# FerrisMind/candle-video

Measured on AMD Instinct MI355X. Metric: frames/sec end-to-end LTX-Video-2B 512x768x97; DiT step ms; VAE decode ms, higher is better.
Workload: dtype bf16; 1 GPU; LTX-Video-0.9.8-2B-distilled 512x768x97, 7 steps (configs.rs:223-240), untiled VAE decode; preset=0.9.8-2b-distilled, denoise_steps=7, parallelism=replicas x1 (no data-path collective)

## Files before the change

candle-video_amd/csrc/gemm_asm.hip:

```cpp
#include <atomic>
#include <cstdlib>
#include <cstring>
#include "gemm_common.h"
#include "options.h"

namespace {

typedef float f32x32 __attribute__((ext_vector_type(32)));
typedef uint32_t u32x16 __attribute__((ext_vector_type(16)));
typedef uint32_t u32x8 __attribute__((ext_vector_type(8)));
typedef uint32_t u32x2 __attribute__((ext_vector_type(2)));
#ifndef GEMM_ASM_LOOP_INC
#define GEMM_ASM_LOOP_INC "gemm_asm_loop.inc"
#endif
#include GEMM_ASM_LOOP_INC

extern __shared__ __attribute__((aligned(16))) unsigned char asm_smem[];

#ifdef LTX_EXPERIMENTS
template <int BM, int BN, int WGM, int WGN> struct AsmLoop;
template <> struct AsmLoop<256, 256, 2, 2> {
    template <typename... T> static __device__ __forceinline__ void run(f32x32 (&c)[10], T&&... t) { gemm_asm_loop_256_256(c[0], c[1], c[2], c[3], c[4], c[5], c[6], c[7], t...); }
};
template <> struct AsmLoop<320, 256, 2, 2> {
    template <typename... T> static __device__ __forceinline__ void run(f32x32 (&c)[10], T&&... t) { gemm_asm_loop_320_256(c[0], c[1], c[2], c[3], c[4], c[5], c[6], c[7], c[8], c[9], t...); }
};
template <> struct AsmLoop<160, 256, 1, 4> {
    template <typename... T> static __device__ __forceinline__ void run(f32x32 (&c)[10], T&&... t) { gemm_asm_loop_160_256(c[0], c[1], c[2], c[3], c[4], t...); }
};

template <int BM, int BN, int WGM, int WGN, int EPI>
__global__ __launch_bounds__(256, 1) void gemm_asm_kernel(const GemmArgs g) {
    constexpr int WM = BM / WGM, WN = BN / WGN, MB = WM / 32, NB = WN / 32, NT = MB * NB, AI = BM / 32, BI = BN / 32;
    constexpr int STAGE = (BM + BN) * 128;
    const int tid = threadIdx.x, lane = tid & 63, wave = __builtin_amdgcn_readfirstlane(tid >> 6);
    const int r = lane & 31, h = lane >> 5;
    const int wm = wave / WGN, wn = wave % WGN;
    const int ntn = (g.N + BN - 1) / BN;
    int bid = blockIdx.x;
    if (g.xcd_remap) {
        const int nblk = (int)gridDim.x, q = nblk >> 3, rr = nblk & 7, x = bid & 7, i = bid >> 3;
        bid = (x < rr ? x * (q + 1) : rr * (q + 1) + (x - rr) * q) + i;
    }
    int mt, nt;
    if (g.group_m > 1) {
        const int ntm = (g.M + BM - 1) / BM, gsz = g.group_m * ntn;
        const int grp = bid / gsz, w = bid - grp * gsz, gm0 = grp * g.group_m;
        const int rows = ntm - gm0 < g.group_m ? ntm - gm0 : g.group_m;
        nt = w / rows; mt = gm0 + (w - nt * rows);
    } else { mt = bid / ntn; nt = bid - mt * ntn; }
    const int m0 = mt * BM, n0 = nt * BN;

#ifndef GEMM_ASM_REG
#define GEMM_ASM_REG 0
#endif
    constexpr bool REGSTAGE = GEMM_ASM_REG && BM == 256 && BN == 256;
// ... 37 lines not shown
    const uint32_t ldsw = (uint32_t)__builtin_amdgcn_readfirstlane((int)(smem_base + (uint32_t)wave * 1024u));
    const int nk = __builtin_amdgcn_readfirstlane(g.K / 64);

    f32x32 c[10];
    AsmLoop<BM, BN, WGM, WGN>::run(c, rbase, dma0, dma1, ra, rw, nk, 0u, 0u, ldsw);

#pragma unroll
    for (int t = 0; t < NT; ++t) {
        const int nb = t / MB, mb = t - nb * MB;
        const int m = m0 + wm * WM + mb * 32 + r;
        if (m >= g.M) continue;
#pragma unroll
        for (int g4 = 0; g4 < 4; ++g4) {
            const int n = n0 + wn * WN + nb * 32 + 8 * g4 + 4 * h;
            if (n >= g.N) continue;
            const int e = (t & 1) * 16 + 4 * g4;
            float v[4] = {c[t >> 1][e], c[t >> 1][e + 1], c[t >> 1][e + 2], c[t >> 1][e + 3]};
            epilogue<bf16_t, EPI>(g, m, n, v);
        }
    }
}

#endif

template <int BM, int BN, int WGM, int WGN> struct AsmLoop16;
template <> struct AsmLoop16<256, 256, 2, 2> {
    template <typename... T> static __device__ __forceinline__ void run(f32x32 (&c)[10], const u32x8& rb, const u32x16& d0, const u32x2&, T&&... t) {
        gemm_asm16_loop_256_256(c[0], c[1], c[2], c[3], c[4], c[5], c[6], c[7], rb, d0, t...); }
    static __device__ __forceinline__ void store(int p, int wm, const f32x32 (&c)[10], const u32x8& ad) {
        if (wm == p) gemm_asm16_store_256_256_p0(c[0], c[1], c[2], c[3], c[4], c[5], c[6], c[7], ad); }
};
template <> struct AsmLoop16<160, 256, 1, 4> {
    template <typename... T> static __device__ __forceinline__ void run(f32x32 (&c)[10], const u32x8& rb, const u32x16& d0, const u32x2&, T&&... t) {
        gemm_asm16_loop_160_256(c[0], c[1], c[2], c[3], c[4], rb, d0, t...); }
    static __device__ __forceinline__ void store(int p, int, const f32x32 (&c)[10], const u32x8& ad) {
        if (p == 0) gemm_asm16_store_160_256_p0(c[0], c[1], c[2], c[3], c[4], ad); else gemm_asm16_store_160_256_p1(c[0], c[1], c[2], c[3], c[4], ad); }
    template <typename... T> static __device__ __forceinline__ void run_res(f32x32 (&c)[10], u32x16 (&res)[5], const u32x2& rvoff, const u32x4& rres, uint32_t rstride,
                                                                            const u32x8& rb, const u32x16& d0, T&&... t) {
        gemm_asm16_loop_160_256_res(c[0], c[1], c[2], c[3], c[4], rb, d0, t..., res[0], res[1], res[2], res[3], res[4], rvoff, rres, rstride); }
};
template <> struct AsmLoop16<320, 256, 2, 2> {
    template <typename... T> static __device__ __forceinline__ void run(f32x32 (&c)[10], const u32x8& rb, const u32x16& d0, const u32x2& d1, T&&... t) {
        gemm_asm16_loop_320_256(c[0], c[1], c[2], c[3], c[4], c[5], c[6], c[7], c[8], c[9], rb, d0, d1, t...); }
    static __device__ __forceinline__ void store(int p, int wm, const f32x32 (&c)[10], const u32x8& ad) {
        if (wm != (p >> 1)) return;
        if ((p & 1) == 0) gemm_asm16_store_320_256_p0(c[0], c[1], c[2], c[3], c[4], c[5], c[6], c[7], c[8], c[9], ad);
        else gemm_asm16_store_320_256_p1(c[0], c[1], c[2], c[3], c[4], c[5], c[6], c[7], c[8], c[9], ad); }
};

#ifdef GEMM_ASM_TRACE
__device__ uint32_t g_asm16_trace[1024 * 4 * 16];
#endif

template <int BM, int BN, int WGM, int WGN, int EPI, bool RSQ = false, bool PF_R = false, bool FOLD = false>
__global__ __launch_bounds__(256, 1) void gemm_asm16_kernel(const GemmArgs g) {
    constexpr int WM = BM / WGM, WN = BN / WGN, MB = WM / 16, NB = WN / 16, NT = MB * NB, AI = BM / 32, BI = BN / 32;
    constexpr int STAGE = (BM + BN) * 128;
#ifdef GEMM_ASM_TRACE
    const uint32_t t_entry = (uint32_t)wall_clock64();
#endif
#ifndef ASM16_NO_KERNARG_BATCH
    asm volatile("" :: "s"(g.A), "s"(g.W), "s"(g.M), "s"(g.N), "s"(g.K), "s"(g.lda), "s"(g.xcd_remap), "s"(g.group_m), "s"(g.rows_per_batch), "s"(gridDim.x));
#endif
    const int tid = threadIdx.x, lane = tid & 63, wave = __builtin_amdgcn_readfirstlane(tid >> 6);
    const int rr = lane & 15, q = lane >> 4;
    const int wm = wave / WGN, wn = wave % WGN;
    const int ntn = (g.N + BN - 1) / BN;
    int bid = blockIdx.x;
    if (g.xcd_remap) {
        const int nblk = (int)gridDim.x, qq = nblk >> 3, r8 = nblk & 7, x = bid & 7, i = bid >> 3;
        bid = (x < r8 ? x * (qq + 1) : r8 * (qq + 1) + (x - r8) * qq) + i;
    }
    int mt, nt;
    if (g.group_m > 1) {
        const int ntm = (g.M + BM - 1) / BM, gsz = g.group_m * ntn;
        const int grp = bid / gsz, w = bid - grp * gsz, gm0 = grp * g.group_m;
        const int rows = ntm - gm0 < g.group_m ? ntm - gm0 : g.group_m;
        nt = w / rows; mt = gm0 + (w - nt * rows);
    } else { mt = bid / ntn; nt = bid - mt * ntn; }
    const int m0 = mt * BM, n0 = nt * BN;
    static_assert(!FOLD || BM <= 256 || BM == 320, "norm fold: 64 extra rows = 256 (row, group) units");
    f32x4 fpt[4], fpx = {0.f, 0.f, 0.f, 0.f};
    if constexpr (FOLD) {
        auto group_of = [&](int row, int q4) {
            const int m = m0 + row < g.M ? m0 + row : g.M - 1;
            const bool in = 4 * q4 < g.rs_n;
            const f32x4 u = *reinterpret_cast<const f32x4*>(g.rs_sq + (int64_t)m * g.rs_n + (in ? 4 * q4 : g.rs_n - 4));
            return in ? u : (f32x4){0.f, 0.f, 0.f, 0.f};
        };
        const int row = tid < BM ? tid : BM - 1;
#pragma unroll
        for (int q4 = 0; q4 < 4; ++q4) fpt[q4] = group_of(row, q4);
        if constexpr (BM > 256) fpx = group_of(256 + (tid >> 2), tid & 3);
    }
    const int lr = lane >> 3, pc = lane & 7;
    u32x16 dma0; u32x2 dma1 = {0x80000000u, 0x80000000u};
#pragma unroll
    for (int j = 0; j < 16; ++j) dma0[j] = 0x80000000u;
    auto set_piece = [&](int j, uint32_t v) { if (j < 16) dma0[j] = v; else dma1[j - 16] = v; };
#pragma unroll
    for (int j = 0; j < AI; ++j) {
        const int row = 8 * (j * 4 + wave) + lr;
        int m = m0 + row; if (m > g.M - 1) m = g.M - 1;
#ifdef ASM16_NOSWZ
        set_piece(j, ((uint32_t)m * (uint32_t)g.lda + (uint32_t)pc * 8u) * 2u);
#else
        set_piece(j, ((uint32_t)m * (uint32_t)g.lda + (uint32_t)(pc ^ ((row >> 1) & 7)) * 8u) * 2u);
#endif
    }
#pragma unroll
    for (int j = 0; j < BI; ++j) {
        const int row = 8 * (j * 4 + wave) + lr;
        int n = n0 + row; if (n > g.N - 1) n = g.N - 1;
#ifdef ASM16_NOSWZ
        set_piece(AI + j, ((uint32_t)n * (uint32_t)g.K + (uint32_t)pc * 8u) * 2u);
#else
        set_piece(AI + j, ((uint32_t)n * (uint32_t)g.K + (uint32_t)(pc ^ ((row >> 1) & 7)) * 8u) * 2u);
#endif
    }
    const uint32_t smem_base = (uint32_t)(uintptr_t)(__attribute__((address_space(3))) unsigned char*)asm_smem;
    u32x8 rbase;
#pragma unroll
    for (int st = 0; st < 2; ++st)
#pragma unroll
        for (int kh = 0; kh < 2; ++kh) {
            const uint32_t ch = (uint32_t)(((4 * kh + q) ^ ((rr >> 1) & 7)) << 4);
            rbase[st * 2 + kh] = smem_base + st * STAGE + BM * 128 + (wn * WN + rr) * 128 + ch;
            rbase[4 + st * 2 + kh] = smem_base + st * STAGE + (wm * WM + rr) * 128 + ch;
        }
    const uint64_t ap = (uint64_t)(uintptr_t)g.A, wp = (uint64_t)(uintptr_t)g.W;
    const u32x4 ra = {(uint32_t)__builtin_amdgcn_readfirstlane((int)(uint32_t)ap), (uint32_t)__builtin_amdgcn_readfirstlane((int)(uint32_t)(ap >> 32)) & 0xffffu, 0x80000000u, 0x00020000u};
    const u32x4 rw = {(uint32_t)__builtin_amdgcn_readfirstlane((int)(uint32_t)wp), (uint32_t)__builtin_amdgcn_readfirstlane((int)(uint32_t)(wp >> 32)) & 0xffffu, 0x80000000u, 0x00020000u};
    const uint32_t ldsw = (uint32_t)__builtin_amdgcn_readfirstlane((int)(smem_base + (uint32_t)wave * 1024u));
    const int nk = __builtin_amdgcn_readfirstlane(g.K / 64);
    f32x32 c[10];
    constexpr bool HAS_R = EPI == EPI_GATE_RESID || EPI == EPI_RESID;
    constexpr int RP = BM == 256 ? 128 : 80;
    static_assert(!PF_R || (HAS_R && BM == 160 && BN == 256), "residual prefetch: the 160 x 256 tile's residual epilogues");
    u32x16 pf[5];
    u32x2 pf_voff = {0x80000000u, 0x80000000u}; u32x4 pf_rsrc = {0u, 0u, 0u, 0u}; uint32_t pf_stride = 0u;
    if constexpr (PF_R) {
        const int rows_valid_pf = g.M - m0 < BM ? g.M - m0 : BM;
        const uint64_t rp = (uint64_t)(uintptr_t)(reinterpret_cast<const bf16_t*>(g.resid) + (int64_t)m0 * g.ldr + n0);
        pf_rsrc = (u32x4){(uint32_t)__builtin_amdgcn_readfirstlane((int)(uint32_t)rp), (uint32_t)__builtin_amdgcn_readfirstlane((int)(uint32_t)(rp >> 32)) & 0xffffu,
                          (uint32_t)__builtin_amdgcn_readfirstlane((int)(((uint32_t)(rows_valid_pf - 1) * (uint32_t)g.ldr + 256u) * 2u)), 0x00020000u};
        const int cg_pf = tid & 31;
        const uint32_t row0 = (uint32_t)(tid >> 5) * (uint32_t)g.ldr * 2u;
        pf_voff[0] = n0 + 4 * cg_pf < g.N ? row0 + (uint32_t)(8 * cg_pf) : 0x80000000u;
        pf_voff[1] = n0 + 4 * cg_pf + 128 < g.N ? row0 + (uint32_t)(8 * cg_pf + 256) : 0x80000000u;
        pf_stride = (uint32_t)__builtin_amdgcn_readfirstlane((int)(8u * (uint32_t)g.ldr * 2u));
    }
    if constexpr (FOLD) {
        __builtin_amdgcn_sched_barrier(0);
        asm volatile("" : "+v"(fpt[0]), "+v"(fpt[1]), "+v"(fpt[2]), "+v"(fpt[3]), "+v"(fpx), "+v"(dma0), "+v"(dma1), "+v"(rbase));
        float* rl = reinterpret_cast<float*>(asm_smem + 2 * STAGE);
        if (tid < BM) {
            float ss = 0.f;
#pragma unroll
            for (int q4 = 0; q4 < 4; ++q4) { ss += fpt[q4][0]; ss += fpt[q4][1]; ss += fpt[q4][2]; ss += fpt[q4][3]; }
            rl[tid] = 1.0f / sqrtf(ss * (1.0f / (float)g.rs_D) + g.rs_eps);
        }
        if constexpr (BM > 256) {
            float run = 0.f;
#pragma unroll
            for (int q4 = 0; q4 < 4; ++q4) {
                const float before = q4 ? __shfl(run, (lane & ~3) + q4 - 1) : 0.f;
                if ((tid & 3) == q4) { run = before; run += fpx[0]; run += fpx[1]; run += fpx[2]; run += fpx[3]; }
            }
            if ((tid & 3) == 3) rl[256 + (tid >> 2)] = 1.0f / sqrtf(run * (1.0f / (float)g.rs_D) + g.rs_eps);
        }
    }
#ifdef ASM16_STAGGER
    const uint32_t k0 = (uint32_t)__builtin_amdgcn_readfirstlane((int)(((unsigned)blockIdx.x % ASM16_STAGGER) * (unsigned)(nk / ASM16_STAGGER) * 128u));
#else
    const uint32_t k0 = 0u;
#endif
#ifdef GEMM_ASM_TRACE
    uint32_t tr[8];
    const uint32_t t_loop0 = (uint32_t)wall_clock64();
    AsmLoop16<BM, BN, WGM, WGN>::run(c, rbase, dma0, dma1, ra, rw, nk, k0, k0, ldsw, (uint32_t)__builtin_amdgcn_readfirstlane(g.K * 2), tr);
    const uint32_t t_loop1 = (uint32_t)wall_clock64();
#else
    if constexpr (PF_R) AsmLoop16<BM, BN, WGM, WGN>::run_res(c, pf, pf_voff, pf_rsrc, pf_stride, rbase, dma0, ra, rw, nk, k0, k0, ldsw, (uint32_t)__builtin_amdgcn_readfirstlane(g.K * 2));
    else AsmLoop16<BM, BN, WGM, WGN>::run(c, rbase, dma0, dma1, ra, rw, nk, k0, k0, ldsw, (uint32_t)__builtin_amdgcn_readfirstlane(g.K * 2));
#endif
// ... 174 lines not shown
                            float* lf = reinterpret_cast<float*>(asm_smem + RP * 1024) + (2 * row) * 36 + cg;
                            lf[0] = lA; lf[36] = lB;
                        } else {
                            float* rowf = reinterpret_cast<float*>(asm_smem + row * 1024);
                            rowf[(cg ^ (row & 15)) << 2] = lA;
                            rowf[((cg + 32) ^ (row & 15)) << 2] = lB;
                        }
                    }
                }
            }
            if constexpr (RSQ) {
                __syncthreads();
                const int ng = (g.N + 127) >> 7;
#pragma unroll 1
                for (int pi = tid; pi < RP * 2; pi += 256) {
                    const int row = pi >> 1, half = pi & 1, sw = row & 15;
                    float sum;
                    if constexpr (RSQ_COMPACT) {
                        const f32x4* lf = reinterpret_cast<const f32x4*>(reinterpret_cast<const float*>(asm_smem + RP * 1024) + pi * 36);
                        f32x4 t[8];
#pragma unroll
                        for (int c4 = 0; c4 < 8; ++c4) t[c4] = lf[c4];
                        sum = t[0][0]; sum += t[0][1]; sum += t[0][2]; sum += t[0][3];
#pragma unroll
                        for (int c4 = 1; c4 < 8; ++c4) { sum += t[c4][0]; sum += t[c4][1]; sum += t[c4][2]; sum += t[c4][3]; }
                    } else {
                        const float* rowf = reinterpret_cast<const float*>(asm_smem + row * 1024);
                        sum = rowf[((32 * half) ^ sw) << 2];
#pragma unroll
                        for (int c2 = 1; c2 < 32; ++c2) sum += rowf[((c2 + 32 * half) ^ sw) << 2];
                    }
                    const int trow = p * RP + row, ncol = n0 + 128 * half;
                    if (m0 + trow < g.M && ncol < g.N) g.rowsq[(int64_t)(m0 + trow) * ng + (ncol >> 7)] = sum;
                }
            }
        }
        };
        if (straddle) run_passes(std::true_type{}); else run_passes(std::false_type{});
#ifdef GEMM_ASM_TRACE
        if (lane == 0 && blockIdx.x < 1024) { uint32_t* o = g_asm16_trace + (blockIdx.x * 4 + wave) * 16; o[13] = t_e0; o[14] = t_e1; o[15] = t_e2; }
#endif
    }
#ifdef GEMM_ASM_TRACE
    asm volatile("s_waitcnt vmcnt(0)" ::: "memory");
    if (lane == 0 && blockIdx.x < 1024) {
        uint32_t* o = g_asm16_trace + (blockIdx.x * 4 + wave) * 16;
        for (int i = 0; i < 8; ++i) o[i] = tr[i];
        uint32_t hwid; asm volatile("s_getreg_b32 %0, hwreg(HW_REG_HW_ID)" : "=s"(hwid));
        o[8] = t_entry; o[9] = t_loop0; o[10] = t_loop1; o[11] = (uint32_t)wall_clock64(); o[12] = hwid;
    }
#endif
}

template <int EPI>
__global__ __launch_bounds__(256, 1) void gemm_asm16_conv_kernel(const GemmArgs g) {
    constexpr int BM = 256, BN = 256, WGN = 2, WM = 128, WN = 128, NB = 8, AI = 8, BI = 8, STAGE = (BM + BN) * 128, RP = 128;
    const int tid = threadIdx.x, lane = tid & 63, wave = __builtin_amdgcn_readfirstlane(tid >> 6);
    const int rr = lane & 15, q = lane >> 4;
    const int wm = wave / WGN, wn = wave % WGN;
    const int ntn = (g.N + BN - 1) / BN;
    const int sf = g.sk_sf > 1 ? g.sk_sf : 1;
    const int tile = (int)blockIdx.x / sf, part = (int)blockIdx.x - tile * sf;
    const int mt = tile / ntn, nt = tile - mt * ntn;
    const int m0 = mt * BM, n0 = nt * BN;
    const int KC = g.Cin / 64, nk = g.ntaps * KC;
    const int kt0 = (int)((int64_t)part * nk / sf), kt1 = (int)((int64_t)(part + 1) * nk / sf);
    const int per_it = 9 * KC, it0 = kt0 / per_it, r2 = kt0 - it0 * per_it, kc0 = r2 / 9, hw0 = r2 - kc0 * 9, ih0 = hw0 / 3, iw0 = hw0 - ih0 * 3;
    const int64_t m_base = m0 > 2 * g.H * g.Wd + g.Wd + 1 ? (int64_t)m0 - (2 * g.H * g.Wd + g.Wd + 1) : 0;
    const int lr = lane >> 3, pc = lane & 7;
    const uint32_t frame_bytes = (uint32_t)g.H * (uint32_t)g.Wd * (uint32_t)g.Cin * 2u;
    u32x16 dma0; u32x8 ab[3], vmask;
#pragma unroll
    for (int j = 0; j < AI; ++j) {
        const int row = 8 * (j * 4 + wave) + lr;
        int m = m0 + row; if (m > g.M - 1) m = g.M - 1;
        const int w = m % g.Wd, t1 = m / g.Wd, h = t1 % g.H, t = (t1 / g.H) % g.T;
        vmask[j] = (uint32_t)((h > 0 ? 1 : 0) | 2 | (h < g.H - 1 ? 4 : 0) | (w > 0 ? 8 : 0) | 16 | (w < g.Wd - 1 ? 32 : 0));
        const uint32_t a_off = ((uint32_t)(m - m_base) * (uint32_t)g.Cin + (uint32_t)(pc ^ ((row >> 1) & 7)) * 8u) * 2u;
#pragma unroll
        for (int i = 0; i < 3; ++i) {
            int tt = t + (it0 + i) - g.pad_t; tt = tt < 0 ? 0 : (tt > g.T - 1 ? g.T - 1 : tt);
            ab[i][j] = a_off + (uint32_t)(tt - t) * frame_bytes;
        }
        dma0[j] = 0x80000000u;
    }
#pragma unroll
    for (int j = 0; j < BI; ++j) {
        const int row = 8 * (j * 4 + wave) + lr;
        int n = n0 + row; if (n > g.N - 1) n = g.N - 1;
        dma0[AI + j] = ((uint32_t)n * (uint32_t)g.K + (uint32_t)(pc ^ ((row >> 1) & 7)) * 8u) * 2u;
    }
    const uint32_t smem_base = (uint32_t)(uintptr_t)(__attribute__((address_space(3))) unsigned char*)asm_smem;
    u32x8 rbase;
#pragma unroll
    for (int st = 0; st < 2; ++st)
#pragma unroll
        for (int kh = 0; kh < 2; ++kh) {
            const uint32_t ch = (uint32_t)(((4 * kh + q) ^ ((rr >> 1) & 7)) << 4);
            rbase[st * 2 + kh] = smem_base + st * STAGE + BM * 128 + (wn * WN + rr) * 128 + ch;
            rbase[4 + st * 2 + kh] = smem_base + st * STAGE + (wm * WM + rr) * 128 + ch;
        }
    const uint64_t ap = (uint64_t)(uintptr_t)(reinterpret_cast<const bf16_t*>(g.A) + m_base * g.Cin), wp = (uint64_t)(uintptr_t)g.W;
    const u32x4 ra = {(uint32_t)__builtin_amdgcn_readfirstlane((int)(uint32_t)ap), (uint32_t)__builtin_amdgcn_readfirstlane((int)(uint32_t)(ap >> 32)) & 0xffffu, 0x80000000u, 0x00020000u};
    const u32x4 rw = {(uint32_t)__builtin_amdgcn_readfirstlane((int)(uint32_t)wp), (uint32_t)__builtin_amdgcn_readfirstlane((int)(uint32_t)(wp >> 32)) & 0xffffu, 0x80000000u, 0x00020000u};
    const uint32_t ldsw = (uint32_t)__builtin_amdgcn_readfirstlane((int)(smem_base + (uint32_t)wave * 1024u));
    const uint32_t cinb = (uint32_t)g.Cin * 2u, rowb = (uint32_t)g.Wd * cinb, nk2 = (uint32_t)g.N * (uint32_t)g.K * 2u;
// ... 94 lines not shown
        __syncthreads();
        if (*flag == 0u) return;
        const float* base = g.sk_ws + (int64_t)tile * sf * (BM * BN);
        constexpr int UR = 4;
#pragma unroll 1
        for (int k0 = 0; k0 < BM / 8; k0 += UR) {
            f32x4 vA[UR], vB[UR];
            bf16x4 qA[UR] = {}, qB[UR] = {};
#pragma unroll
            for (int j = 0; j < UR; ++j) {
                const int trow = r0 + 8 * (k0 + j);
                int m = m0 + trow; if (m > g.M - 1) m = g.M - 1;
                const float* rp = base + trow * BN + 4 * cg;
                vA[j] = *reinterpret_cast<const f32x4*>(rp); vB[j] = *reinterpret_cast<const f32x4*>(rp + 128);
                if constexpr (EPI == EPI_RESID) {
                    const bf16_t* rrow = reinterpret_cast<const bf16_t*>(g.resid) + (int64_t)m * g.ldr;
                    if (nA < g.N) qA[j] = *reinterpret_cast<const bf16x4*>(rrow + nA);
                    if (nB < g.N) qB[j] = *reinterpret_cast<const bf16x4*>(rrow + nB);
                }
            }
            for (int pq = 1; pq < sf; ++pq) {
#pragma unroll
                for (int j = 0; j < UR; ++j) {
                    const float* rp = base + (int64_t)pq * (BM * BN) + (r0 + 8 * (k0 + j)) * BN + 4 * cg;
                    vA[j] += *reinterpret_cast<const f32x4*>(rp); vB[j] += *reinterpret_cast<const f32x4*>(rp + 128);
                }
            }
#pragma unroll
            for (int j = 0; j < UR; ++j) {
                const int m = m0 + r0 + 8 * (k0 + j);
                if (m >= g.M) continue;
                float a4[4] = {vA[j][0], vA[j][1], vA[j][2], vA[j][3]}, b4[4] = {vB[j][0], vB[j][1], vB[j][2], vB[j][3]};
                if constexpr (EPI == EPI_D2S) {
                    if (nA < g.N) epilogue<bf16_t, EPI>(g, m, nA, a4);
                    if (nB < g.N) epilogue<bf16_t, EPI>(g, m, nB, b4);
                } else {
                    bf16_t* crow = reinterpret_cast<bf16_t*>(g.C) + (int64_t)m * g.ldc;
                    if (nA < g.N) {
                        for (int i = 0; i < 4; ++i) a4[i] += bA4[i];
                        if constexpr (EPI == EPI_RESID) for (int i = 0; i < 4; ++i) a4[i] += (float)qA[j][i];
                        store4<bf16_t>(crow + nA, a4);
                    }
                    if (nB < g.N) {
                        for (int i = 0; i < 4; ++i) b4[i] += bB4[i];
                        if constexpr (EPI == EPI_RESID) for (int i = 0; i < 4; ++i) b4[i] += (float)qB[j][i];
                        store4<bf16_t>(crow + nB, b4);
                    }
                }
            }
        }
    }
}

struct AsmTile { int bm, bn; const char* name; };
const AsmTile kAsmTiles[] = {{256, 256, "asm256x256"}, {320, 256, "asm320x256"}, {160, 256, "asm160x256"}};

template <int BM, int BN, int WGM, int WGN, int EPI, bool MF16 = false>
int launch_asm(const GemmArgs& g, hipStream_t s) {
    constexpr int smem = 2 * (BM + BN) * 128;
    static std::atomic<unsigned long long> attr_devs{0}, attr_devs_rsq{0};
    void (*kern)(const GemmArgs);
#ifdef LTX_EXPERIMENTS
    if constexpr (MF16) kern = gemm_asm16_kernel<BM, BN, WGM, WGN, EPI>; else kern = gemm_asm_kernel<BM, BN, WGM, WGN, EPI>;
#else
    static_assert(MF16, "the 32x32x16 kernel is an experiment build's");
    kern = gemm_asm16_kernel<BM, BN, WGM, WGN, EPI>;
#endif
    bool wrote_rowsq = false;
    constexpr bool CAN_PF = MF16 && BM == 160 && BN == 256 && (EPI == EPI_GATE_RESID || EPI == EPI_RESID);
    bool pf_r = false;
    if constexpr (CAN_PF) pf_r = g.K / 64 >= 12 && ltx_exp("gemm_asm16_resid_prefetch", 1);
    if constexpr (MF16 && (EPI == EPI_BIAS || EPI == EPI_GATE_RESID || EPI == EPI_RESID)) {
        if (g.rowsq) { kern = gemm_asm16_kernel<BM, BN, WGM, WGN, EPI, true>; wrote_rowsq = true; }
    }
    static std::atomic<unsigned long long> attr_devs_pf{0}, attr_devs_pf_rsq{0};
    if constexpr (CAN_PF) {
        if (pf_r) kern = g.rowsq ? gemm_asm16_kernel<BM, BN, WGM, WGN, EPI, true, true> : gemm_asm16_kernel<BM, BN, WGM, WGN, EPI, false, true>;
    }
    static std::atomic<unsigned long long> attr_devs_fold{0};
    bool fold_in = false;
    if constexpr (MF16 && (EPI == EPI_BIAS || EPI == EPI_GELU)) {
        if (g.rs_sq) {
            if (g.rowsq || !g.cvec || g.rs_n < 4 || g.rs_n > 16 || g.rs_n % 4 || g.rows_per_batch < 1) LTX_FAIL(LTX_ERR_ARG, "gemm_asm16: norm fold needs cvec, 4 .. 16 row partials in groups of four and no rowsq by-product");
            kern = gemm_asm16_kernel<BM, BN, WGM, WGN, EPI, false, false, true>; fold_in = true;
        }
    } else if (g.rs_sq) LTX_FAIL(LTX_ERR_ARG, "gemm_asm16: norm fold (rs_sq) on an epilogue that does not carry it");
    if (g.C2 && !(wrote_rowsq && (EPI == EPI_GATE_RESID || EPI == EPI_RESID))) LTX_FAIL(LTX_ERR_ARG, "gemm_asm16: the second output (C2) rides on the residual epilogues with rowsq");
    const int smem_l = smem + (fold_in ? 2048 : 0);
    LTX_TRY(ltx_set_max_dyn_smem(fold_in ? attr_devs_fold : pf_r ? (wrote_rowsq ? attr_devs_pf_rsq : attr_devs_pf) : (wrote_rowsq ? attr_devs_rsq : attr_devs), reinterpret_cast<const void*>(kern), smem_l));
    GemmArgs ga = g;
    ga.xcd_remap = ltx_exp("xcd_remap", 1);
    {
        const int C = 32;
        int gm = 1; while ((gm + 1) * (gm + 1) * BM <= C * BN) ++gm;
        { const int x_gm = ltx_exp("gemm_group_m", -1); if (x_gm >= 0) gm = x_gm; }
        const int ntm = cdiv(g.M, BM);
        if (gm > ntm) gm = ntm;
        ga.group_m = gm < 2 ? 0 : gm;
    }
    const int tiles = cdiv(g.M, BM) * cdiv(g.N, BN);
    LTX_LAUNCH_TIMED(kern, dim3((unsigned)tiles), dim3(256), smem_l, s, ga);
    LTX_CHECK_LAUNCH();
    if (wrote_rowsq) ltx_gemm_rowsq_done();
    return LTX_OK;
}

template <int BM, int BN, int WGM, int WGN, bool MF16 = false>
int launch_asm_epi(const GemmArgs& g, int epi, hipStream_t s) {
    switch (epi) {
        case EPI_BIAS: return launch_asm<BM, BN, WGM, WGN, EPI_BIAS, MF16>(g, s);
        case EPI_GELU: return launch_asm<BM, BN, WGM, WGN, EPI_GELU, MF16>(g, s);
        case EPI_GATE_RESID: return launch_asm<BM, BN, WGM, WGN, EPI_GATE_RESID, MF16>(g, s);
        case EPI_RESID: return launch_asm<BM, BN, WGM, WGN, EPI_RESID, MF16>(g, s);
    }
    LTX_FAIL(LTX_ERR_ARG, "gemm_asm: bad epilogue");
}

}

bool ltx_gemm_asm16_fits(const GemmArgs& g, int epi) {
    if (g.conv || g.pn_on) return false;
    if (epi != EPI_BIAS && epi != EPI_GELU && epi != EPI_GATE_RESID && epi != EPI_RESID) return false;
    if (g.K < 128 || g.K % 64 != 0 || g.lda % 8 != 0 || ((uintptr_t)g.A & 15) || ((uintptr_t)g.W & 15)) return false;
    if ((double)g.M * g.lda * 2.0 >= 2147483648.0 || (double)g.N * g.K * 2.0 >= 2147483648.0) return false;
    const bool seg_ok = !g.c_seg_shift || ((1 << g.c_seg_shift) % 256 == 0 && g.c_seg_stride % 4 == 0);
    if ((double)g.ldc * 2.0 * 320.0 >= 2147483648.0 || (double)g.ldr * 2.0 * 320.0 >= 2147483648.0) return false;
    if (g.N % 8 != 0 || g.ldc % 4 != 0 || ((uintptr_t)g.C & 7) || !seg_ok) return false;
    if (g.bias && ((uintptr_t)g.bias & 7)) return false;
    if ((epi == EPI_GATE_RESID || epi == EPI_RESID) && (!g.resid || g.ldr % 4 != 0 || ((uintptr_t)g.resid & 7))) return false;
    if (epi == EPI_GATE_RESID && (!g.gate || ((uintptr_t)g.gate & 15) || g.gate_stride % 4 != 0 || g.rows_per_batch < 320)) return false;
    if (ltx_gemm_split_factor(g) > 1) return false;
    return g.M > 512 && g.N >= 512;
}

bool ltx_gemm_fold_ok(const GemmArgs& g, int epi) {
    if (!ltx_gemm_asm16_fits(g, epi) || (ltx_opt().gemm_off & LTX_FAM_ASM16) || !ltx_opt().gemm_wide_epi) return false;
    if (ltx_gemm_route_kind(g, LTX_DT_BF16, epi) != LTX_ROUTE_PLAN) return false;
    if (g.C2) {
        if ((epi != EPI_GATE_RESID && epi != EPI_RESID) || !g.rowsq || !g.scale2 || g.scale2_stride % 4 || ((uintptr_t)g.scale2 & 15) || ((uintptr_t)g.C2 & 7) || g.rows_per_batch < 320 || g.c_seg_shift) return false;
    }
    if (g.rs_sq) {
        if ((epi != EPI_BIAS && epi != EPI_GELU) || g.rowsq || !g.cvec || g.cvec_stride % 4 || ((uintptr_t)g.cvec & 15) || g.rs_n < 4 || g.rs_n > 16 || g.rs_n % 4 || ((uintptr_t)g.rs_sq & 15) || g.rows_per_batch < 320) return false;
    }
    return true;
}

bool ltx_gemm_asm_eligible(const GemmArgs& g, int dtype, int epi) {
#ifdef LTX_EXPERIMENTS
    if (dtype != LTX_DT_BF16 || g.conv || ltx_exp("gemm_asm", 0) != 1) return false;
    if (epi != EPI_BIAS && epi != EPI_GELU && epi != EPI_GATE_RESID && epi != EPI_RESID) return false;
    if (g.K < 128 || g.K % 64 != 0 || g.lda % 8 != 0 || ((uintptr_t)g.A & 15) || ((uintptr_t)g.W & 15)) return false;
    if ((double)g.M * g.lda * 2.0 >= 2147483648.0 || (double)g.N * g.K * 2.0 >= 2147483648.0) return false;
    if (ltx_gemm_split_factor(g) > 1) return false;
    return g.M >= 2048 && g.N >= 1024;
#else
    (void)g; (void)dtype; (void)epi;
    return false;
#endif
}

int ltx_gemm_asm_pick_tile(int M, int N) {
    { const int f = ltx_exp("gemm_asm_tile", -1); if (f >= 0 && f < 3) return f; }
    double best = 1e30; int bi = 0;
    for (int i = 0; i < 3; ++i) {
        const int64_t tiles = (int64_t)cdiv(M, kAsmTiles[i].bm) * cdiv(N, kAsmTiles[i].bn);
        const double cost = (double)cdiv64(tiles, 256) * (double)(kAsmTiles[i].bm * kAsmTiles[i].bn);
        if (cost < best * 0.999) { best = cost; bi = i; }
    }
    return bi;
}
const char* ltx_gemm_asm_tile_name(int i) { return i >= 0 && i < 3 ? kAsmTiles[i].name : ""; }

#ifdef GEMM_ASM_TRACE
extern "C" int ltx_dbg_gemm_asm16_trace(uint32_t* out, int n_words) {
    return hipMemcpyFromSymbol(out, HIP_SYMBOL(g_asm16_trace), (size_t)n_words * 4) == hipSuccess ? 0 : -1;
}
#endif

int ltx_launch_gemm_asm16(const GemmArgs& g, int epi, int tile, hipStream_t s) {
    if (((epi == EPI_GATE_RESID && g.gate) || g.C2 || g.rs_sq) && g.rows_per_batch < 320)
        LTX_FAIL(LTX_ERR_ARG, "gemm_asm16: per-group epilogue vectors need groups of at least 320 rows (a tile may meet one group boundary)");
    ltx_prof_kernel(LTX_PROFK_GEMM_ASM16);
    switch (tile) {
        case 0: return launch_asm_epi<256, 256, 2, 2, true>(g, epi, s);
        case 1: return launch_asm_epi<320, 256, 2, 2, true>(g, epi, s);
        case 2: return launch_asm_epi<160, 256, 1, 4, true>(g, epi, s);
    }
    LTX_FAIL(LTX_ERR_ARG, "gemm_asm16: unsupported tile");
}

bool ltx_gemm_asm16_conv_fits(const GemmArgs& g, int epi) {
    if (!g.conv || g.ntaps != 27 || g.kh != 3 || g.kw != 3 || g.pn_on || g.c_seg_shift || g.rowsq) return false;
    if (epi != EPI_BIAS && epi != EPI_RESID && epi != EPI_D2S) return false;
    if (g.Cin % 64 != 0 || g.K != g.Cin || g.N % 8 != 0 || ((uintptr_t)g.A & 15) || ((uintptr_t)g.W & 15) || ((uintptr_t)g.C & 7)) return false;
    if (g.bias && ((uintptr_t)g.bias & 7)) return false;
    if (epi == EPI_RESID && (!g.resid || g.ldr % 4 != 0 || ((uintptr_t)g.resid & 7) || g.ldc % 4 != 0)) return false;
    if (epi == EPI_BIAS && g.ldc % 4 != 0) return false;
    if (epi == EPI_D2S && (g.Cf % 4 != 0 || g.N != 8 * g.Cf)) return false;
    if ((double)g.N * g.K * 2.0 * 10.0 >= 4294967296.0) return false;
    return g.M > 512 && g.N >= 1024 && ltx_gemm_big_fits(g);
}

int ltx_launch_gemm_asm16_conv(const GemmArgs& g, int epi, hipStream_t s) {
    if (!ltx_gemm_asm16_conv_fits(g, epi)) LTX_FAIL(LTX_ERR_ARG, "gemm_asm16 (conv): shape not eligible");
    ltx_prof_kernel(LTX_PROFK_GEMM_ASM16);
    constexpr int smem = 2 * (256 + 256) * 128;
    static std::atomic<unsigned long long> devs[3] = {{0}, {0}, {0}};
    void (*kern)(const GemmArgs) = epi == EPI_BIAS ? gemm_asm16_conv_kernel<EPI_BIAS> : (epi == EPI_RESID ? gemm_asm16_conv_kernel<EPI_RESID> : gemm_asm16_conv_kernel<EPI_D2S>);
    LTX_TRY(ltx_set_max_dyn_smem(devs[epi == EPI_BIAS ? 0 : (epi == EPI_RESID ? 1 : 2)], reinterpret_cast<const void*>(kern), smem));
    GemmArgs ga = g;
    const int tiles = cdiv(g.M, 256) * cdiv(g.N, 256);
    LTX_TRY(ltx_gemm_split_workspace(&ga, tiles, 256, 256, s));
    const int sf = ga.sk_sf > 1 ? ga.sk_sf : 1;
    LTX_LAUNCH_TIMED(kern, dim3((unsigned)(tiles * sf)), dim3(256), smem, s, ga);
    LTX_CHECK_LAUNCH();
    return LTX_OK;
}

int ltx_launch_gemm_asm(const GemmArgs& g, int epi, hipStream_t s) {
#ifdef LTX_EXPERIMENTS
    ltx_prof_kernel(LTX_PROFK_GEMM_ASM);
    switch (ltx_gemm_asm_pick_tile(g.M, g.N)) {
        case 0: return launch_asm_epi<256, 256, 2, 2>(g, epi, s);
        case 1: return launch_asm_epi<320, 256, 2, 2>(g, epi, s);
// ... 8 lines not shown
```

candle-video_amd/csrc/options.cpp:

```cpp
#include "options.h"
#include <atomic>
#include <cstdio>
#include <cstdlib>
#include <cstring>
#include <map>
#include <mutex>
#include <string>
#include "errors.h"

namespace {
std::mutex g_mu;
LtxOptions g_opt;
std::atomic<bool> g_loaded{false};
std::map<std::string, int> g_exp;

struct ListBit { const char* name; unsigned bit; };
const ListBit kFam[] = {{"asm16", LTX_FAM_ASM16}, {"ring", LTX_FAM_RING}, {"p8", LTX_FAM_P8}, {"halo", LTX_FAM_HALO}, {"halo_out", LTX_FAM_HALO_OUT}, {"big", LTX_FAM_BIG}};
const ListBit kAttn[] = {{"q64", LTX_ATTN_Q64}, {"q128", LTX_ATTN_Q128}, {"cross", LTX_ATTN_CROSS}, {"pipe", LTX_ATTN_PIPE}};

template <size_t N> bool parse_list(const char* v, const ListBit (&tab)[N], unsigned* out) {
    unsigned bits = 0;
    std::string s(v ? v : "");
    size_t p = 0;
    while (p < s.size()) {
        size_t q = s.find('+', p); if (q == std::string::npos) q = s.size();
        const std::string item = s.substr(p, q - p);
        bool ok = item.empty();
        for (const auto& t : tab) if (item == t.name) { bits |= t.bit; ok = true; }
        if (!ok) return false;
        p = q + 1;
    }
    *out = bits;
    return true;
}

struct IntField { const char* name; int LtxOptions::*field; };
const IntField kInts[] = {
    {"gemm_tune", &LtxOptions::gemm_tune}, {"gemm_wide_epi", &LtxOptions::gemm_wide_epi}, {"gemm_trace", &LtxOptions::gemm_trace},
    {"attn_q64_big", &LtxOptions::attn_q64_big}, {"vae_tile_batch", &LtxOptions::vae_tile_batch}, {"prof_kernel_events", &LtxOptions::prof_kernel_events}, {"ff2_defer", &LtxOptions::ff2_defer},
    {"gemm_splitk", &LtxOptions::gemm_splitk}, {"q2_fold", &LtxOptions::q2_fold}, {"norm_presum", &LtxOptions::norm_presum}, {"norm_lean", &LtxOptions::norm_lean},
    {"xattn_compact", &LtxOptions::xattn_compact}, {"dense_qkv", &LtxOptions::dense_qkv}, {"vae_fuse_norm", &LtxOptions::vae_fuse_norm}, {"t5_attn_mfma", &LtxOptions::t5_attn_mfma}, {"guidance_batch", &LtxOptions::guidance_batch}, {"norm_fold", &LtxOptions::norm_fold}, {"norm_fold_copies", &LtxOptions::norm_fold_copies}, {"attn_q64_stream", &LtxOptions::attn_q64_stream},
};

bool set_one(LtxOptions& o, const std::string& key, const char* value) {
    static const LtxOptions dflt;
    for (const auto& f : kInts) if (key == f.name) {
        if (!value) { o.*(f.field) = dflt.*(f.field); return true; }
        char* end = nullptr; const long v = strtol(value, &end, 10);
        if (end == value || *end) return false;
        o.*(f.field) = (int)v; return true;
    }
    if (key == "gemm_plan") {
        if (!value) { o.gemm_plan[0] = 0; return true; }
        if (strlen(value) >= sizeof(o.gemm_plan)) return false;
        strcpy(o.gemm_plan, value); return true;
    }
    if (key == "gemm_off") return value ? parse_list(value, kFam, &o.gemm_off) : (o.gemm_off = 0, true);
    if (key == "attn_off") return value ? parse_list(value, kAttn, &o.attn_off) : (o.attn_off = 0, true);
    if (key.rfind("x_", 0) == 0) {
        if (!value) { g_exp.erase(key); return true; }
        char* end = nullptr; const long v = strtol(value, &end, 10);
        if (end == value || *end) return false;
        g_exp[key] = (int)v; return true;
    }
    return false;
}

bool parse_string(LtxOptions& o, const char* text, std::string* bad) {
    std::string s(text ? text : "");
    size_t p = 0;
    while (p < s.size()) {
        size_t q = s.find(',', p); if (q == std::string::npos) q = s.size();
        const std::string item = s.substr(p, q - p);
        p = q + 1;
        if (item.empty()) continue;
        const size_t eq = item.find('=');
        if (eq == std::string::npos || !set_one(o, item.substr(0, eq), item.c_str() + eq + 1)) { if (bad) *bad = item; return false; }
    }
    return true;
}

void load_locked() {
    g_opt = LtxOptions(); g_exp.clear();
    std::string bad;
    if (!parse_string(g_opt, getenv("LTX_OPTIONS"), &bad))
        fprintf(stderr, "[ltx] LTX_OPTIONS: entry '%s' not understood (see include/ltxhip.h); it and what follows it are ignored\n", bad.c_str());
    g_loaded.store(true, std::memory_order_release);
}
}

const LtxOptions& ltx_opt() {
// ... 51 lines not shown
```

candle-video_amd/csrc/options.h:

```cpp
#pragma once

enum { LTX_FAM_ASM16 = 1, LTX_FAM_RING = 2, LTX_FAM_P8 = 4, LTX_FAM_HALO = 8, LTX_FAM_HALO_OUT = 16, LTX_FAM_BIG = 32 };
enum { LTX_ATTN_Q64 = 1, LTX_ATTN_Q128 = 2, LTX_ATTN_CROSS = 4, LTX_ATTN_PIPE = 8 };

struct LtxOptions {
    int gemm_tune = 1;
    char gemm_plan[40] = {0};
    unsigned gemm_off = 0;
    int gemm_wide_epi = 1;
    int gemm_trace = 0;
    int attn_q64_big = -1;
    int vae_tile_batch = 0;
    int prof_kernel_events = 1;
    int ff2_defer = 1;
    int gemm_splitk = 1;
    int q2_fold = 1;
    int norm_presum = 1;
    int norm_lean = 1;
    int xattn_compact = 1;
    int attn_q64_stream = 0;
    int norm_fold = 2;
    int norm_fold_copies = 10;
    int guidance_batch = 1;
    int dense_qkv = 1;
    int vae_fuse_norm = 1;
    int t5_attn_mfma = 1;
    unsigned attn_off = 0;
};

const LtxOptions& ltx_opt();
int ltx_exp_lookup(const char* name, int dflt);
#ifdef LTX_EXPERIMENTS
#define ltx_exp(name, dflt) ltx_exp_lookup(name, dflt)
#else
#define ltx_exp(name, dflt) (dflt)
#endif
```

Before: 541.5 frames/sec.

## Run two GEMM tiles per workgroup when tile count exceeds CU count

Splits the asm16 GEMM kernel body into a per-tile device function and adds a paired launch mode. When there are more tiles than CUs, each workgroup processes up to two tiles in sequence, and the grid is halved. In paired mode the buffer descriptors are rebased to each tile's origin with a tight record size. The aim is to cut launch and wave-quantisation tail overhead, at the cost of serialising two tiles per workgroup and adding a barrier between them.

```diff
diff --git a/candle-video_amd/csrc/gemm_asm.hip b/candle-video_amd/csrc/gemm_asm.hip
--- a/candle-video_amd/csrc/gemm_asm.hip
+++ b/candle-video_amd/csrc/gemm_asm.hip
@@ -2,6 +2,7 @@
 #include <cstdlib>
 #include <cstring>
 #include "gemm_common.h"
+#include "gemm_pair.h"
 #include "options.h"
 
 namespace {
@@ -145,32 +146,21 @@
 __device__ uint32_t g_asm16_trace[1024 * 4 * 16];
 #endif
 
-template <int BM, int BN, int WGM, int WGN, int EPI, bool RSQ = false, bool PF_R = false, bool FOLD = false>
-__global__ __launch_bounds__(256, 1) void gemm_asm16_kernel(const GemmArgs g) {
+template <int BM, int BN, int WGM, int WGN, int EPI, bool RSQ, bool PF_R, bool FOLD, bool ORIGIN>
+__device__ __forceinline__ void gemm_asm16_tile(const GemmArgs& g, const int pos, const int nblk) {
     constexpr int WM = BM / WGM, WN = BN / WGN, MB = WM / 16, NB = WN / 16, NT = MB * NB, AI = BM / 32, BI = BN / 32;
     constexpr int STAGE = (BM + BN) * 128;
 #ifdef GEMM_ASM_TRACE
     const uint32_t t_entry = (uint32_t)wall_clock64();
 #endif
-#ifndef ASM16_NO_KERNARG_BATCH
-    asm volatile("" :: "s"(g.A), "s"(g.W), "s"(g.M), "s"(g.N), "s"(g.K), "s"(g.lda), "s"(g.xcd_remap), "s"(g.group_m), "s"(g.rows_per_batch), "s"(gridDim.x));
-#endif
-    const int tid = threadIdx.x, lane = tid & 63, wave = __builtin_amdgcn_readfirstlane(tid >> 6);
+    int tid_ = threadIdx.x;
+    if constexpr (ORIGIN) asm volatile("" : "+v"(tid_));
+    const int tid = tid_, lane = tid & 63, wave = __builtin_amdgcn_readfirstlane(tid >> 6);
     const int rr = lane & 15, q = lane >> 4;
     const int wm = wave / WGN, wn = wave % WGN;
     const int ntn = (g.N + BN - 1) / BN;
-    int bid = blockIdx.x;
-    if (g.xcd_remap) {
-        const int nblk = (int)gridDim.x, qq = nblk >> 3, r8 = nblk & 7, x = bid & 7, i = bid >> 3;
-        bid = (x < r8 ? x * (qq + 1) : r8 * (qq + 1) + (x - r8) * qq) + i;
-    }
     int mt, nt;
-    if (g.group_m > 1) {
-        const int ntm = (g.M + BM - 1) / BM, gsz = g.group_m * ntn;
-        const int grp = bid / gsz, w = bid - grp * gsz, gm0 = grp * g.group_m;
-        const int rows = ntm - gm0 < g.group_m ? ntm - gm0 : g.group_m;
-        nt = w / rows; mt = gm0 + (w - nt * rows);
-    } else { mt = bid / ntn; nt = bid - mt * ntn; }
+    ltx_tile_of_position(pos, nblk, (g.M + BM - 1) / BM, ntn, g.group_m, g.xcd_remap, &mt, &nt);
     const int m0 = mt * BM, n0 = nt * BN;
     static_assert(!FOLD || BM <= 256 || BM == 320, "norm fold: 64 extra rows = 256 (row, group) units");
     f32x4 fpt[4], fpx = {0.f, 0.f, 0.f, 0.f};
@@ -195,6 +185,7 @@
     for (int j = 0; j < AI; ++j) {
         const int row = 8 * (j * 4 + wave) + lr;
         int m = m0 + row; if (m > g.M - 1) m = g.M - 1;
+        if constexpr (ORIGIN) m = row;
 #ifdef ASM16_NOSWZ
         set_piece(j, ((uint32_t)m * (uint32_t)g.lda + (uint32_t)pc * 8u) * 2u);
 #else
@@ -205,6 +196,7 @@
     for (int j = 0; j < BI; ++j) {
         const int row = 8 * (j * 4 + wave) + lr;
         int n = n0 + row; if (n > g.N - 1) n = g.N - 1;
+        if constexpr (ORIGIN) n = row;
 #ifdef ASM16_NOSWZ
         set_piece(AI + j, ((uint32_t)n * (uint32_t)g.K + (uint32_t)pc * 8u) * 2u);
 #else
@@ -221,9 +213,12 @@
             rbase[st * 2 + kh] = smem_base + st * STAGE + BM * 128 + (wn * WN + rr) * 128 + ch;
             rbase[4 + st * 2 + kh] = smem_base + st * STAGE + (wm * WM + rr) * 128 + ch;
         }
-    const uint64_t ap = (uint64_t)(uintptr_t)g.A, wp = (uint64_t)(uintptr_t)g.W;
-    const u32x4 ra = {(uint32_t)__builtin_amdgcn_readfirstlane((int)(uint32_t)ap), (uint32_t)__builtin_amdgcn_readfirstlane((int)(uint32_t)(ap >> 32)) & 0xffffu, 0x80000000u, 0x00020000u};
-    const u32x4 rw = {(uint32_t)__builtin_amdgcn_readfirstlane((int)(uint32_t)wp), (uint32_t)__builtin_amdgcn_readfirstlane((int)(uint32_t)(wp >> 32)) & 0xffffu, 0x80000000u, 0x00020000u};
+    const uint64_t ap = (uint64_t)(uintptr_t)(reinterpret_cast<const bf16_t*>(g.A) + (ORIGIN ? (int64_t)m0 * g.lda : 0));
+    const uint64_t wp = (uint64_t)(uintptr_t)(reinterpret_cast<const bf16_t*>(g.W) + (ORIGIN ? (int64_t)n0 * g.K : 0));
+    const uint32_t a_rec = ORIGIN ? ((uint32_t)((g.M - m0 < BM ? g.M - m0 : BM) - 1) * (uint32_t)g.lda + (uint32_t)g.K) * 2u : 0x80000000u;
+    const uint32_t w_rec = ORIGIN ? ((uint32_t)((g.N - n0 < BN ? g.N - n0 : BN) - 1) * (uint32_t)g.K + (uint32_t)g.K) * 2u : 0x80000000u;
+    const u32x4 ra = {(uint32_t)__builtin_amdgcn_readfirstlane((int)(uint32_t)ap), (uint32_t)__builtin_amdgcn_readfirstlane((int)(uint32_t)(ap >> 32)) & 0xffffu, (uint32_t)__builtin_amdgcn_readfirstlane((int)a_rec), 0x00020000u};
+    const u32x4 rw = {(uint32_t)__builtin_amdgcn_readfirstlane((int)(uint32_t)wp), (uint32_t)__builtin_amdgcn_readfirstlane((int)(uint32_t)(wp >> 32)) & 0xffffu, (uint32_t)__builtin_amdgcn_readfirstlane((int)w_rec), 0x00020000u};
     const uint32_t ldsw = (uint32_t)__builtin_amdgcn_readfirstlane((int)(smem_base + (uint32_t)wave * 1024u));
     const int nk = __builtin_amdgcn_readfirstlane(g.K / 64);
     f32x32 c[10];
@@ -504,6 +499,26 @@
 #endif
 }
 
+template <int BM, int BN, int WGM, int WGN, int EPI, bool RSQ = false, bool PF_R = false, bool FOLD = false, bool TWO = false>
+__global__ __launch_bounds__(256, 1) void gemm_asm16_kernel(const GemmArgs g) {
+#ifndef ASM16_NO_KERNARG_BATCH
+    asm volatile("" :: "s"(g.A), "s"(g.W), "s"(g.M), "s"(g.N), "s"(g.K), "s"(g.lda), "s"(g.xcd_remap), "s"(g.group_m), "s"(g.rows_per_batch), "s"(gridDim.x));
+#endif
+    if constexpr (!TWO) {
+        gemm_asm16_tile<BM, BN, WGM, WGN, EPI, RSQ, PF_R, FOLD, false>(g, (int)blockIdx.x, (int)gridDim.x);
+    } else {
+        static_assert(!PF_R && BM != 160, "pair form: the two-round tiles");
+        const int tiles = ((g.M + BM - 1) / BM) * ((g.N + BN - 1) / BN), groups = (int)gridDim.x;
+#pragma unroll 1
+        for (int which = 0; which < 2; ++which) {
+            const int pos = ltx_pair_position((int)blockIdx.x, which, groups, tiles);
+            if (pos < 0) break;
+            if (which) __syncthreads();
+            gemm_asm16_tile<BM, BN, WGM, WGN, EPI, RSQ, PF_R, FOLD, true>(g, pos, tiles);
+        }
+    }
+}
+
 template <int EPI>
 __global__ __launch_bounds__(256, 1) void gemm_asm16_conv_kernel(const GemmArgs g) {
     constexpr int BM = 256, BN = 256, WGN = 2, WM = 128, WN = 128, NB = 8, AI = 8, BI = 8, STAGE = (BM + BN) * 128, RP = 128;
@@ -704,6 +719,20 @@
     }
 }
 
+int asm16_n_cu() {
+    static std::atomic<int> per_dev[64];
+    int dev = 0; if (hipGetDevice(&dev) != hipSuccess || dev < 0 || dev >= 64) return 256;
+    int n = per_dev[dev].load(std::memory_order_relaxed);
+    if (n == 0) {
+        n = 256;
+        int v = 0; if (hipDeviceGetAttribute(&v, hipDeviceAttributeMultiprocessorCount, dev) == hipSuccess && v > 0) n = v;
+        per_dev[dev].store(n, std::memory_order_relaxed);
+    }
+    return n;
+}
+
+std::atomic<unsigned long long> g_pair_launches{0};
+
 struct AsmTile { int bm, bn; const char* name; };
 const AsmTile kAsmTiles[] = {{256, 256, "asm256x256"}, {320, 256, "asm320x256"}, {160, 256, "asm160x256"}};
 
@@ -751,7 +780,24 @@
         ga.group_m = gm < 2 ? 0 : gm;
     }
     const int tiles = cdiv(g.M, BM) * cdiv(g.N, BN);
-    LTX_LAUNCH_TIMED(kern, dim3((unsigned)tiles), dim3(256), smem_l, s, ga);
+    bool paired = false;
+    if constexpr (MF16 && BM != 160) {
+        paired = ltx_pair_wanted(ltx_opt().gemm_two_tile, tiles, asm16_n_cu()) && tiles > 1 && g.K >= 192 && g.lda >= g.K;
+        if (paired) {
+            static std::atomic<unsigned long long> attr_devs_two{0}, attr_devs_two_rsq{0}, attr_devs_two_fold{0};
+            std::atomic<unsigned long long>* devs = &attr_devs_two;
+            kern = gemm_asm16_kernel<BM, BN, WGM, WGN, EPI, false, false, false, true>;
+            if constexpr (EPI == EPI_BIAS || EPI == EPI_GATE_RESID || EPI == EPI_RESID) {
+                if (wrote_rowsq) { kern = gemm_asm16_kernel<BM, BN, WGM, WGN, EPI, true, false, false, true>; devs = &attr_devs_two_rsq; }
+            }
+            if constexpr (EPI == EPI_BIAS || EPI == EPI_GELU) {
+                if (fold_in) { kern = gemm_asm16_kernel<BM, BN, WGM, WGN, EPI, false, false, true, true>; devs = &attr_devs_two_fold; }
+            }
+            LTX_TRY(ltx_set_max_dyn_smem(*devs, reinterpret_cast<const void*>(kern), smem_l));
+            g_pair_launches.fetch_add(1, std::memory_order_relaxed);
+        }
+    }
+    LTX_LAUNCH_TIMED(kern, dim3((unsigned)ltx_pair_groups(tiles, paired)), dim3(256), smem_l, s, ga);
     LTX_CHECK_LAUNCH();
     if (wrote_rowsq) ltx_gemm_rowsq_done();
     return LTX_OK;
@@ -822,6 +868,8 @@
     return bi;
 }
 const char* ltx_gemm_asm_tile_name(int i) { return i >= 0 && i < 3 ? kAsmTiles[i].name : ""; }
+
+extern "C" unsigned long long ltx_dbg_gemm_pair_launches(void) { return g_pair_launches.load(std::memory_order_relaxed); }
 
 #ifdef GEMM_ASM_TRACE
 extern "C" int ltx_dbg_gemm_asm16_trace(uint32_t* out, int n_words) {
diff --git a/candle-video_amd/csrc/gemm_pair.h b/candle-video_amd/csrc/gemm_pair.h
--- /dev/null
+++ b/candle-video_amd/csrc/gemm_pair.h
@@ -0,0 +1,27 @@
+#pragma once
+
+#if defined(__HIPCC__) || defined(__CUDACC__)
+#define LTX_PAIR_HD __host__ __device__ __forceinline__
+#else
+#define LTX_PAIR_HD inline
+#endif
+
+LTX_PAIR_HD bool ltx_pair_wanted(int mode, int tiles, int n_cu) { return mode == 2 || (mode == 1 && tiles > n_cu); }
+LTX_PAIR_HD int ltx_pair_groups(int tiles, bool paired) { return paired ? (tiles + 1) / 2 : tiles; }
+LTX_PAIR_HD int ltx_pair_position(int w, int which, int groups, int tiles) {
+    const int pos = w + which * groups;
+    return pos < tiles ? pos : -1;
+}
+LTX_PAIR_HD void ltx_tile_of_position(int pos, int nblk, int ntm, int ntn, int group_m, int xcd_remap, int* mt, int* nt) {
+    int bid = pos;
+    if (xcd_remap) {
+        const int qq = nblk >> 3, r8 = nblk & 7, x = bid & 7, i = bid >> 3;
+        bid = (x < r8 ? x * (qq + 1) : r8 * (qq + 1) + (x - r8) * qq) + i;
+    }
+    if (group_m > 1) {
+        const int gsz = group_m * ntn;
+        const int grp = bid / gsz, w = bid - grp * gsz, gm0 = grp * group_m;
+        const int rows = ntm - gm0 < group_m ? ntm - gm0 : group_m;
+        *nt = w / rows; *mt = gm0 + (w - *nt * rows);
+    } else { *mt = bid / ntn; *nt = bid - *mt * ntn; }
+}
diff --git a/candle-video_amd/csrc/options.cpp b/candle-video_amd/csrc/options.cpp
--- a/candle-video_amd/csrc/options.cpp
+++ b/candle-video_amd/csrc/options.cpp
@@ -36,7 +36,7 @@
 
 struct IntField { const char* name; int LtxOptions::*field; };
 const IntField kInts[] = {
-    {"gemm_tune", &LtxOptions::gemm_tune}, {"gemm_wide_epi", &LtxOptions::gemm_wide_epi}, {"gemm_trace", &LtxOptions::gemm_trace},
+    {"gemm_tune", &LtxOptions::gemm_tune}, {"gemm_wide_epi", &LtxOptions::gemm_wide_epi}, {"gemm_trace", &LtxOptions::gemm_trace}, {"gemm_two_tile", &LtxOptions::gemm_two_tile},
     {"attn_q64_big", &LtxOptions::attn_q64_big}, {"vae_tile_batch", &LtxOptions::vae_tile_batch}, {"prof_kernel_events", &LtxOptions::prof_kernel_events}, {"ff2_defer", &LtxOptions::ff2_defer},
     {"gemm_splitk", &LtxOptions::gemm_splitk}, {"q2_fold", &LtxOptions::q2_fold}, {"norm_presum", &LtxOptions::norm_presum}, {"norm_lean", &LtxOptions::norm_lean},
     {"xattn_compact", &LtxOptions::xattn_compact}, {"dense_qkv", &LtxOptions::dense_qkv}, {"vae_fuse_norm", &LtxOptions::vae_fuse_norm}, {"t5_attn_mfma", &LtxOptions::t5_attn_mfma}, {"guidance_batch", &LtxOptions::guidance_batch}, {"norm_fold", &LtxOptions::norm_fold}, {"norm_fold_copies", &LtxOptions::norm_fold_copies}, {"attn_q64_stream", &LtxOptions::attn_q64_stream},
diff --git a/candle-video_amd/csrc/options.h b/candle-video_amd/csrc/options.h
--- a/candle-video_amd/csrc/options.h
+++ b/candle-video_amd/csrc/options.h
@@ -8,6 +8,7 @@
     char gemm_plan[40] = {0};
     unsigned gemm_off = 0;
     int gemm_wide_epi = 1;
+    int gemm_two_tile = 1;
     int gemm_trace = 0;
     int attn_q64_big = -1;
     int vae_tile_batch = 0;
```

After: 543.4 frames/sec, median of 6. Within noise of the previous version (+0.4%).
